# nunofachada/cl_ops

Hardware: AMD Instinct MI355X
Metric: Mkeys/s sorting 2^28 uint32 (satradix, 4-bit digits); achieved % of HBM roofline (higher is better)
Workload: dtype u32

## Files before the change

cl_ops_amd/csrc/hip/clo_hip_internal.h:

```cpp
#ifndef CLO_HIP_INTERNAL_H
#define CLO_HIP_INTERNAL_H

#include <stddef.h>
#include <stdint.h>

#include "clo_hip.h"

#define CLO_WS_STATUS_OFFSET 0
#define CLO_WS_EPOCH_WORD    2
#define CLO_WS_DONE_WORD     3
#define CLO_WS_TICKET_WORD   16
#define CLO_WS_MAX_PASSES    64
#define CLO_WS_HEADER_BYTES  512

struct clo_hip_env_t { unsigned max_spins; int radix_sweep; int r1_pools; int no_digits; int bitonic_merge2; };
const clo_hip_env_t* clo_hip_env();
int clo_radixw_preload();

inline bool clo_misaligned(const void* p, size_t align) { return ((uintptr_t) p & (align - 1)) != 0; }
inline bool clo_ws_misaligned(const void* ws) { return clo_misaligned(ws, CLO_HIP_WORKSPACE_ALIGN); }

#ifdef __HIPCC__
#include <hip/hip_runtime.h>

void clo_timing_begin(const char* label, hipStream_t s);
void clo_timing_end(hipStream_t s);
struct clo_timing_scope {
	hipStream_t s;
	clo_timing_scope(const char* label, hipStream_t stream) : s(stream) { clo_timing_begin(label, s); }
	~clo_timing_scope() { clo_timing_end(s); }
};

struct clo_keyx {
	unsigned long long sign, field;
	int kind;
};
template <typename E>
__device__ __forceinline__ E clo_keyx_fwd(E x, const clo_keyx& k) {
	if (k.kind == 1) return (E) (x ^ (E) k.sign);
	if (k.kind == 2) return (E) (x ^ ((x & (E) k.sign) ? (E) k.field : (E) k.sign));
	return x;
}
template <typename E>
__device__ __forceinline__ E clo_keyx_inv(E x, const clo_keyx& k) {
	if (k.kind == 1) return (E) (x ^ (E) k.sign);
	if (k.kind == 2) return (E) (x ^ ((x & (E) k.sign) ? (E) k.sign : (E) k.field));
	return x;
}
inline clo_keyx clo_keyx_make(int kind, int key_shift, int key_bits) {
	clo_keyx k = { 0, 0, 0 };
	if (kind == 1 || kind == 2) {
		k.kind = kind;
		k.sign = 1ull << (key_shift + key_bits - 1);
		k.field = (key_bits >= 64 ? ~0ull : ((1ull << key_bits) - 1ull)) << key_shift;
	}
	return k;
}

struct clo_kv_io {
	const void* keys_in;
	const unsigned* values_in;
	void* keys_out;
	unsigned* values_out;
};

size_t clo_radix4_workspace_bytes(size_t n, int elem_size, int digit_bits, int key_bits);
int clo_radix4_sort_kv(const clo_kv_io& io, void* pairs_a, void* pairs_b, size_t n, int key_size, int key_shift,
	int key_bits, int digit_bits, clo_keyx kx, void* ws, hipStream_t s);
size_t clo_radix4_partition_workspace_bytes(size_t n, int elem_size, int bits);
int clo_radix4_partition(const void* src, void* dst, size_t n, int elem_size, unsigned shift, int bits,
	unsigned long long* counts, void* ws, hipStream_t s);
int clo_radix4_sort(const void* src, void* dst, void* tmp, size_t n, int elem_size, int key_shift,
	int key_bits, int digit_bits, clo_keyx kx, const unsigned char* first_dig, void* ws, hipStream_t s);
int clo_radix4_takes_first_digits(size_t n, int elem_size, int digit_bits);
size_t clo_radix4_lds_bytes(int elem_size, int digit_bits);
int clo_radix1_applies(size_t n, int elem_size, int digit_bits);
size_t clo_radix1_workspace_bytes(size_t n, int elem_size, int key_bits);
int clo_radix1_sort(const void* src, void* dst, void* tmp, size_t n, int elem_size, int key_shift, int key_bits,
	clo_keyx kx, void* ws, unsigned* status, hipStream_t s);
int clo_bitonic_tiled_e1(void* data, size_t numel, int key_shift, int key_bits, int key_size, int key_kind, int descending, int* launches, hipStream_t s);
int clo_bitonic_tiled_e2(void* data, size_t numel, int key_shift, int key_bits, int key_size, int key_kind, int descending, int* launches, hipStream_t s);
int clo_bitonic_tiled_e4(void* data, size_t numel, int key_shift, int key_bits, int key_size, int key_kind, int descending, int* launches, hipStream_t s);
int clo_bitonic_tiled_e8(void* data, size_t numel, int key_shift, int key_bits, int key_size, int key_kind, int descending, int* launches, hipStream_t s);
size_t clo_radixw_lds_bytes(int digit_bits);
struct clo_radix_counters { unsigned* thist; unsigned* toff; unsigned* partial; unsigned* tinfo; unsigned tiles; bool big; };
int clo_radixw_launch_tilehist(const void* in, size_t n, int elem_size, int bits, unsigned shift, unsigned mask,
	const clo_radix_counters& c, clo_keyx kx, hipStream_t s);
int clo_radixw_launch_tilehist_kv(const void* keys, size_t n, int key_size, int bits, unsigned shift, unsigned mask,
	const clo_radix_counters& c, clo_keyx kx, hipStream_t s);
int clo_radixw_launch_tilehist_bytes(const unsigned char* dig, size_t n, int elem_size, int bits, unsigned mask,
	const clo_radix_counters& c, hipStream_t s);
int clo_radixw_launch_offsets(int bits, const clo_radix_counters& c, const unsigned** dbase, hipStream_t s);
size_t clo_radixw_partial_rows(size_t tiles);

#define CLO_SEG_MAX 256
struct clo_seg_tile { unsigned in_base, count_seg, out_base, seg_n; };
struct clo_seg_chunk { unsigned t0, tend, c_first, seg_last; };
struct clo_seg_pieces {
// ... 95 lines not shown
```

cl_ops_amd/csrc/hip/clo_hip_radix4.hip:

```cpp
#include <hip/hip_runtime.h>

#include <cstdlib>
#include <type_traits>

#include "clo_hip.h"
#include "clo_hip_internal.h"
#include "clo_hip_radix_rank.h"

namespace {

template <int KB> struct kv_key;
template <> struct kv_key<1> { typedef uint8_t type; };
template <> struct kv_key<2> { typedef uint16_t type; };
template <> struct kv_key<4> { typedef uint32_t type; };

template <int KB, int ITEMS>
__device__ __forceinline__ void kv_load_pairs(const clo_kv_io& kv, size_t at, unsigned valid, bool aligned, uint64_t (&pair)[ITEMS]) {
	typedef typename kv_key<KB>::type K;
	const K* kp = reinterpret_cast<const K*>(kv.keys_in) + at;
	K k[ITEMS];
	unsigned v[ITEMS];
	if (valid == (unsigned) ITEMS) {
		load_blocked<K, ITEMS>(kp, k, aligned);
		if (kv.values_in) {
			load_blocked<unsigned, ITEMS>(kv.values_in + at, v, aligned);
		} else {
			#pragma unroll
			for (int i = 0; i < ITEMS; ++i) v[i] = (unsigned) at + (unsigned) i;
		}
	} else {
		#pragma unroll
		for (int i = 0; i < ITEMS; ++i) {
			k[i] = (unsigned) i < valid ? kp[i] : (K) 0;
			v[i] = (unsigned) i < valid ? (kv.values_in ? kv.values_in[at + i] : (unsigned) at + (unsigned) i) : 0u;
		}
	}
	#pragma unroll
	for (int i = 0; i < ITEMS; ++i) pair[i] = ((uint64_t) k[i] << 32) | v[i];
}

template <int KB>
__device__ __forceinline__ void kv_store_pair(const clo_kv_io& kv, unsigned gi, uint64_t e) {
	typedef typename kv_key<KB>::type K;
	if (kv.keys_out) reinterpret_cast<K*>(kv.keys_out)[gi] = (K) (e >> 32);
	kv.values_out[gi] = (unsigned) e;
}

template <typename E, int LB, int HB, bool BIG, bool DIG = false, bool SEG = false, int KV_IN = 0, int KV_OUT = 0>
__global__ __launch_bounds__((pair_shape<E, BIG>::THREADS), (pair_shape<E, BIG>::THREADS >= 1024 ? 8 : 6))
void clo_radix4_pair_kernel(const E* __restrict__ in, E* __restrict__ out, size_t n,
	unsigned shift, unsigned mask_lo, unsigned mask_hi,
	const unsigned* __restrict__ thist, const unsigned* __restrict__ toff, const unsigned* __restrict__ dbase,
	const unsigned* __restrict__ tinfo, int aligned,
	clo_keyx kx_in, clo_keyx kx_out, unsigned char* __restrict__ dig_out = nullptr, unsigned next_shift = 0,
	const clo_seg_tile* __restrict__ tdesc = nullptr, const E* __restrict__ in2 = nullptr, clo_kv_io kv = clo_kv_io()) {
	static_assert((KV_IN == 0 && KV_OUT == 0) || (sizeof(E) == 8 && !SEG), "key-value passes: 8-byte pairs, one array");

	constexpr int THREADS = pair_shape<E, BIG>::THREADS;
	constexpr int ITEMS = pair_shape<E, BIG>::ITEMS;
	constexpr int TILE = THREADS * ITEMS;
	constexpr int WAVES = THREADS / 64;
	constexpr int R2 = 1 << (LB + HB);
	constexpr int HMAX = pc_words<(LB > HB ? LB : HB)>::H;
	static_assert(R2 <= 256 && R2 <= THREADS, "one thread per combined digit, scanned by the first four waves");

	__shared__ __attribute__((aligned(16))) E s_stage[TILE];
	constexpr bool ALIAS = pair_shape<E, BIG>::ALIAS;
	__shared__ unsigned s_end[ALIAS ? 1 : THREADS * PC_END_STRIDE];
	__shared__ unsigned s_wtot[WAVES][HMAX];
	__shared__ __attribute__((aligned(16))) unsigned s_wbase[WAVES][HMAX];
	__shared__ unsigned s_delta[R2];
	__shared__ unsigned s_w4[4];

	const unsigned tid = threadIdx.x, lane = tid & 63u, wave = tid >> 6;
	const unsigned per_xcd = SEG ? (unsigned) ((n + 7) / 8) : (unsigned) ((n + (size_t) TILE * 8 - 1) / ((size_t) TILE * 8));
	const unsigned tile = (blockIdx.x & 7u) * per_xcd + (blockIdx.x >> 3);
	size_t base = (size_t) tile * TILE;
	unsigned count, n32;
	if constexpr (SEG) {
		if (tile >= (unsigned) n) return;
		const clo_seg_tile td = tdesc[tile];
		base = (size_t) td.in_base;
		count = td.count_seg & 0xffffu;
		n32 = td.seg_n;
		out += td.out_base;
		if constexpr (DIG) dig_out += td.out_base;
		dbase += (size_t) ((td.count_seg >> 16) & 0x7fffu) * R2;
		if (td.count_seg >> 31) in = in2;
	} else {
		if (base >= n) return;
		count = (n - base) < (size_t) TILE ? (unsigned) (n - base) : (unsigned) TILE;
		n32 = n > 0xffffffffull ? 0xffffffffu : (unsigned) n;
	}
	const bool full = count == (unsigned) TILE;
	const unsigned tbase = tid * ITEMS;
	const unsigned mask2 = (mask_hi << LB) | mask_lo;

	__builtin_amdgcn_s_setprio(3);
	unsigned h2 = 0, goff = 0;
	if (tid < (unsigned) R2) {
		h2 = thist[(size_t) tile * R2 + tid];
		goff = toff[(size_t) tile * R2 + tid];
		if (dbase) goff += dbase[tid];
	}
	E key[ITEMS];
	if constexpr (KV_IN != 0) {
		kv_load_pairs<KV_IN, ITEMS>(kv, base + tbase, full ? (unsigned) ITEMS : (count > tbase ? count - tbase : 0u), aligned != 0, key);
	} else if (full) {
		if constexpr (SEG) load_blocked_unaligned<E, ITEMS>(in + base + tbase, key);
		else load_blocked<E, ITEMS>(in + base + tbase, key, aligned != 0);
	} else {
		#pragma unroll
		for (int i = 0; i < ITEMS; ++i) key[i] = (tbase + i < count) ? in[base + tbase + i] : (E) 0;
	}
	__builtin_amdgcn_s_setprio(0);
	if (kx_in.kind) {
		#pragma unroll
		for (int i = 0; i < ITEMS; ++i) key[i] = clo_keyx_fwd<E>(key[i], kx_in);
	}
	{
		const unsigned incl2 = clo_wave_scan_inclusive<unsigned>(h2, lane);
		if (lane == 63 && wave < 4) s_w4[wave] = incl2;
		if (tid < (unsigned) R2) s_delta[tid] = goff - (incl2 - h2);
	}

	const bool single = tinfo[tile] != 0u;

	if (!single) {
		pc_local_split<E, LB, THREADS, ITEMS, HMAX, pc_no_mid, pc_no_counted, ALIAS>(key, shift, mask_lo, count, s_stage, s_end, s_wtot, s_wbase);
	} else {
		if (full) {
			constexpr int PER = ITEMS * (int) sizeof(E) >= 16 ? 16 / (int) sizeof(E) : ITEMS;
			typedef E vec16 __attribute__((ext_vector_type(PER)));
			#pragma unroll
			for (int k = 0; k < ITEMS / PER; ++k) {
				vec16 t;
				#pragma unroll
				for (int q = 0; q < PER; ++q) t[q] = key[k * PER + q];
				*reinterpret_cast<vec16*>(&s_stage[tbase + k * PER]) = t;
			}
		} else {
			#pragma unroll
			for (int i = 0; i < ITEMS; ++i) if (tbase + i < count) s_stage[tbase + i] = key[i];
		}
		clo_lds_barrier();
	}

	if (tid < (unsigned) R2) {
		unsigned before = 0;
		#pragma unroll
		for (unsigned w = 0; w < 4; ++w) if (w < wave) before += s_w4[w];
		s_delta[tid] -= before;
	}
	if (single) {
		__syncthreads();
	} else if (mask_hi != 0) {
		if (full) {
			constexpr int PER = ITEMS * (int) sizeof(E) >= 16 ? 16 / (int) sizeof(E) : ITEMS;
			typedef E vec16 __attribute__((ext_vector_type(PER)));
			#pragma unroll
			for (int k = 0; k < ITEMS / PER; ++k) {
				const vec16 t = *reinterpret_cast<const vec16*>(&s_stage[tbase + k * PER]);
				#pragma unroll
				for (int q = 0; q < PER; ++q) key[k * PER + q] = t[q];
			}
		} else {
			#pragma unroll
			for (int i = 0; i < ITEMS; ++i) if (tbase + i < count) key[i] = s_stage[tbase + i];
		}
		pc_local_split<E, HB, THREADS, ITEMS, HMAX, pc_no_mid, pc_no_counted, ALIAS>(key, shift + LB, mask_hi, count, s_stage, s_end, s_wtot, s_wbase);
	} else {
		__syncthreads();
	}

	constexpr int VEC = sizeof(E) >= 8 ? 1 : 4;
	typedef E vecE __attribute__((ext_vector_type(VEC)));
	typedef E vecE_u __attribute__((ext_vector_type(VEC), aligned(sizeof(E))));
	const bool dig_bytes = DIG && VEC == 4 && (next_shift & 7u) == 0u && next_shift < 8u * (unsigned) sizeof(E);
	const unsigned dig_b = next_shift >> 3;
	const unsigned dig_sel_lo = 0x0c0c0400u + dig_b * 0x0101u, dig_sel_hi = 0x04000c0cu + dig_b * 0x01010000u;
	const unsigned nbits2 = (unsigned) __builtin_popcount(mask2);
	const auto scatter = [&](auto kx_tag) {
		constexpr bool KX = decltype(kx_tag)::value;
		#pragma unroll
		for (int j = 0; j < ITEMS / VEC; ++j) {
			const unsigned p = (j * THREADS + tid) * VEC;
			if (full) {
				const vecE v = *reinterpret_cast<const vecE*>(&s_stage[p]);
				const unsigned d0 = pc_digit<E>(v[0], shift, mask2, nbits2), dl = pc_digit<E>(v[VEC - 1], shift, mask2, nbits2);
				const unsigned gi0 = p + s_delta[d0];
				if (d0 == dl && gi0 <= n32 - VEC) {
					vecE vo = v;
					if constexpr (KX) {
						#pragma unroll
						for (int k = 0; k < VEC; ++k) vo[k] = clo_keyx_inv<E>(v[k], kx_out);
					}
					if constexpr (KV_OUT != 0) kv_store_pair<KV_OUT>(kv, gi0, vo[0]);
					else *reinterpret_cast<vecE_u*>(&out[gi0]) = vo;
					if constexpr (DIG) {
						if constexpr (VEC == 4) {
							typedef unsigned u32_u __attribute__((aligned(1)));
							unsigned dg;
							if (dig_bytes)
								dg = __builtin_amdgcn_perm((unsigned) v[1], (unsigned) v[0], dig_sel_lo) | __builtin_amdgcn_perm((unsigned) v[3], (unsigned) v[2], dig_sel_hi);
							else
								dg = ((unsigned) (v[0] >> next_shift) & 255u) | (((unsigned) (v[1] >> next_shift) & 255u) << 8)
									| (((unsigned) (v[2] >> next_shift) & 255u) << 16) | ((unsigned) (v[3] >> next_shift) << 24);
							*reinterpret_cast<u32_u*>(dig_out + gi0) = dg;
						} else {
							dig_out[gi0] = (unsigned char) (v[0] >> next_shift);
						}
					}
				} else {
					#pragma unroll
					for (int k = 0; k < VEC; ++k) {
						const unsigned gi = p + k + s_delta[pc_digit<E>(v[k], shift, mask2, nbits2)];
						if (gi < n32) {
							if constexpr (KV_OUT != 0) kv_store_pair<KV_OUT>(kv, gi, KX ? clo_keyx_inv<E>(v[k], kx_out) : v[k]);
							else out[gi] = KX ? clo_keyx_inv<E>(v[k], kx_out) : v[k];
							if constexpr (DIG) dig_out[gi] = (unsigned char) (v[k] >> next_shift);
						}
					}
				}
			} else {
				#pragma unroll
				for (int k = 0; k < VEC; ++k) {
					if (p + k < count) {
						const E e = s_stage[p + k];
						const unsigned gi = p + k + s_delta[pc_digit<E>(e, shift, mask2, nbits2)];
						if (gi < n32) {
							if constexpr (KV_OUT != 0) kv_store_pair<KV_OUT>(kv, gi, KX ? clo_keyx_inv<E>(e, kx_out) : e);
							else out[gi] = KX ? clo_keyx_inv<E>(e, kx_out) : e;
							if constexpr (DIG) dig_out[gi] = (unsigned char) (e >> next_shift);
						}
					}
				}
			}
		}
	};
	if (kx_out.kind) scatter(std::true_type()); else scatter(std::false_type());
}

constexpr int SMALL_TILE = 512 * 8;
template <typename E> struct small_big { static constexpr int THREADS = 1024, ITEMS = sizeof(E) == 8 ? 8 : 16, TILE = THREADS * ITEMS; };

template <typename E, int BITS, int THREADS, int ITEMS>
__global__ __launch_bounds__(THREADS)
void clo_radix4_small_kernel(const E* in, E* out, unsigned n, unsigned key_shift, unsigned key_bits, clo_keyx kx) {
	constexpr int H = pc_words<BITS>::H;
	constexpr int WAVES = THREADS / 64;
	__shared__ __attribute__((aligned(16))) E s_stage[THREADS * ITEMS];
	__shared__ unsigned s_end[THREADS * PC_END_STRIDE];
	__shared__ unsigned s_wtot[WAVES][H];
	__shared__ __attribute__((aligned(16))) unsigned s_wbase[WAVES][H];

	const unsigned tbase = threadIdx.x * ITEMS;
	E key[ITEMS];
	#pragma unroll
	for (int i = 0; i < ITEMS; ++i) key[i] = (tbase + i < n) ? clo_keyx_fwd<E>(in[tbase + i], kx) : (E) 0;
	for (unsigned done = 0; done < key_bits; done += BITS) {
		const unsigned bits = key_bits - done < (unsigned) BITS ? key_bits - done : (unsigned) BITS;
		pc_local_split<E, BITS, THREADS, ITEMS, H>(key, key_shift + done, (1u << bits) - 1u, n,
			s_stage, s_end, s_wtot, s_wbase);
		if constexpr (ITEMS * sizeof(E) >= 16) {
			constexpr int PER = 16 / (int) sizeof(E);
			typedef E vec16 __attribute__((ext_vector_type(PER)));
			#pragma unroll
			for (int k = 0; k < ITEMS / PER; ++k) {
				const vec16 t = *reinterpret_cast<const vec16*>(&s_stage[tbase + k * PER]);
				#pragma unroll
				for (int q = 0; q < PER; ++q) key[k * PER + q] = t[q];
			}
		} else {
			#pragma unroll
			for (int i = 0; i < ITEMS; ++i) if (tbase + i < n) key[i] = s_stage[tbase + i];
		}
	}
	#pragma unroll
	for (int i = 0; i < ITEMS; ++i) if (tbase + i < n) out[tbase + i] = clo_keyx_inv<E>(key[i], kx);
}


struct rp_layout { size_t thist, toff, partial, tinfo, dig, total, tiles; bool big; };

rp_layout rp_make_layout(size_t n, int elem_size, int pass_bits, bool digits = true) {
	rp_layout L;
	const size_t R2 = (size_t) 1 << pass_bits;
	L.big = clo_radix_big_tiles(n, elem_size);
	const size_t tile = clo_pair_tile_elems(elem_size, L.big);
	L.tiles = (n + tile - 1) / tile;
	if (L.tiles == 0) L.tiles = 1;
	const size_t per = L.tiles * R2 * sizeof(unsigned);
	L.thist = CLO_WS_HEADER_BYTES;
	L.toff = L.thist + per;
	L.partial = L.toff + per;
	L.tinfo = L.partial + ((clo_radixw_partial_rows(L.tiles) * R2 * sizeof(unsigned) + 255) & ~(size_t) 255);
	L.total = L.tinfo + ((L.tiles * sizeof(unsigned) + 255) & ~(size_t) 255);
	L.dig = 0;
	if (digits && clo_radix_digit_stream(n, elem_size)) {
		L.dig = L.total;
		L.total += (n + 255) & ~(size_t) 255;
	}
	return L;
}

template <typename Layout>
clo_radix_counters rp_counters(void* ws, const Layout& L, size_t tiles) {
	char* w = (char*) ws;
	return { (unsigned*) (w + L.thist), (unsigned*) (w + L.toff), (unsigned*) (w + L.partial), (unsigned*) (w + L.tinfo), (unsigned) tiles, L.big };
}

struct rp_digits { unsigned shift, mask_lo, mask_hi, mask, next_shift; };

template <int LB, int HB>
rp_digits rp_pass_digits(int p, int key_shift, int key_bits) {
	constexpr int PB = LB + HB;
	const int rem = key_bits - p * PB;
	const int bits = rem < PB ? rem : PB;
	const int lo_bits = bits < LB ? bits : LB, hi_bits = bits - lo_bits;
	rp_digits d;
	d.shift = (unsigned) (key_shift + p * PB);
	d.mask_lo = (1u << lo_bits) - 1u;
	d.mask_hi = (1u << hi_bits) - 1u;
	d.mask = (d.mask_hi << LB) | d.mask_lo;
	d.next_shift = d.shift + PB;
	return d;
}

template <typename E, int LB, int HB, bool SEG = false, int KB = 0>
void rp_launch_pass(const clo_radix_counters& c, const rp_digits& d, const E* in, E* out, size_t n, const unsigned* dbase, int aligned,
	clo_keyx kx_in, clo_keyx kx_out, unsigned char* dig_out, hipStream_t s, const clo_seg_tile* tdesc = nullptr, const E* in2 = nullptr,
	bool kv_in = false, bool kv_out = false, const clo_kv_io& kv = clo_kv_io()) {
	const unsigned tiles = SEG ? (unsigned) n : c.tiles;
	const auto launch = [&](auto big, auto dig, auto kvi, auto kvo) {
		constexpr bool BIG = decltype(big)::value, DIG = decltype(dig)::value;
		hipLaunchKernelGGL((clo_radix4_pair_kernel<E, LB, HB, BIG, DIG, SEG, decltype(kvi)::value, decltype(kvo)::value>),
			dim3((tiles + 7u) / 8u * 8u), dim3(pair_shape<E, BIG>::THREADS), 0, s,
			in, out, n, d.shift, d.mask_lo, d.mask_hi, c.thist, c.toff, dbase, c.tinfo, aligned, kx_in, kx_out, dig_out, d.next_shift, tdesc, in2, kv);
	};
	const auto shape = [&](auto kvi, auto kvo) {
		constexpr bool BIG_OK = sizeof(E) >= 4, DIG_OK = BIG_OK && LB == 4 && HB == 4 && decltype(kvo)::value == 0;
		if constexpr (DIG_OK) {
			if (c.big && dig_out) { launch(std::true_type(), std::true_type(), kvi, kvo); return; }
		}
		if constexpr (BIG_OK) {
			if (c.big) { launch(std::true_type(), std::false_type(), kvi, kvo); return; }
		}
		launch(std::false_type(), std::false_type(), kvi, kvo);
	};
	typedef std::integral_constant<int, 0> plain;
	typedef std::integral_constant<int, KB> key;
	if (kv_in && kv_out) shape(key(), key());
	else if (kv_in) shape(key(), plain());
	else if (kv_out) shape(plain(), key());
	else shape(plain(), plain());
}

int kv_unpack(const uint64_t* pairs, const clo_kv_io& io, size_t n, int key_size, hipStream_t s);

template <typename E, int LB, int HB, int KB = 0>
int rp_sort_impl(const E* src, E* dst, E* tmp, size_t n, int key_shift, int key_bits, clo_keyx kx, const unsigned char* first_dig,
	const clo_kv_io& kv, void* ws, hipStream_t s) {
	constexpr int PB = LB + HB;
	const int passes = (key_bits + PB - 1) / PB;
	const rp_layout L = rp_make_layout(n, (int) sizeof(E), PB);
	const clo_radix_counters c = rp_counters(ws, L, L.tiles);
	const bool no_dig = clo_hip_env()->no_digits != 0;
	constexpr bool DIG_OK = LB == 4 && HB == 4 && sizeof(E) >= 4;
	unsigned char* dig = (DIG_OK && L.dig != 0 && passes > 1 && !no_dig) ? (unsigned char*) ws + L.dig : nullptr;
	const clo_keyx kx_none = { 0, 0, 0 };
	const bool split_after = KB != 0 && passes == 1 && (kv.keys_out == kv.keys_in || (const void*) kv.values_out == (const void*) kv.values_in);
	const bool kv_aligned = (uintptr_t) kv.keys_in % 16 == 0 && (uintptr_t) kv.values_in % 16 == 0;

	hipError_t e;

	const bool inplace_odd = (dst == src) && (passes % 2 == 1);
	const E* cur_in = src;
	for (int p = 0; p < passes; ++p) {
		E* cur_out;
		if (inplace_odd) cur_out = (p % 2 == 0) ? tmp : dst;
		else cur_out = ((passes - 1 - p) % 2 == 0) ? dst : tmp;
		const bool kv_in = KB != 0 && p == 0, kv_out = KB != 0 && p + 1 == passes && !split_after;
		const rp_digits d = rp_pass_digits<LB, HB>(p, key_shift, key_bits);
		{
			clo_timing_scope timing("radix_hist", s);
			const unsigned char* hist_bytes = (dig && p > 0) ? dig : ((DIG_OK && c.big && p == 0 && kx.kind == 0) ? first_dig : nullptr);
			const int st = kv_in ? clo_radixw_launch_tilehist_kv(kv.keys_in, n, KB, PB, d.shift, d.mask, c, kx, s)
				: hist_bytes ? clo_radixw_launch_tilehist_bytes(hist_bytes, n, (int) sizeof(E), PB, d.mask, c, s)
				: clo_radixw_launch_tilehist(cur_in, n, (int) sizeof(E), PB, d.shift, d.mask, c, p == 0 ? kx : kx_none, s);
			if (st != 0) return st;
		}
		const unsigned* dbase = nullptr;
		{
			clo_timing_scope timing("radix_offsets", s);
			const int st = clo_radixw_launch_offsets(PB, c, &dbase, s);
			if (st != 0) return st;
		}
		{
			clo_timing_scope timing("radix_pass", s);
			const int aligned = kv_in ? (int) kv_aligned : (int) ((uintptr_t) cur_in % 16 == 0);
			rp_launch_pass<E, LB, HB, false, KB>(c, d, cur_in, cur_out, n, dbase, aligned, p == 0 ? kx : kx_none, p + 1 == passes ? kx : kx_none,
				p + 1 < passes ? dig : nullptr, s, nullptr, nullptr, kv_in, kv_out, kv);
		}
		cur_in = cur_out;
	}
	e = hipGetLastError();
	if (e != hipSuccess) return (int) e;
	if (inplace_odd) {
		e = hipMemcpyAsync(dst, tmp, n * sizeof(E), hipMemcpyDeviceToDevice, s);
		if (e != hipSuccess) return (int) e;
	}
	if constexpr (KB != 0) {
		if (split_after) return kv_unpack(dst, kv, n, KB, s);
	}
	return 0;
}

template <typename E>
int rp_dispatch(const void* src, void* dst, void* tmp, size_t n, int key_shift, int key_bits, int digit_bits,
	clo_keyx kx, const unsigned char* first_dig, void* ws, hipStream_t s) {
	#define CLO_RP(LB, HB) return rp_sort_impl<E, LB, HB>((const E*) src, (E*) dst, (E*) tmp, n, key_shift, key_bits, kx, first_dig, clo_kv_io(), ws, s)
	switch (digit_bits) {
		case 1: CLO_RP(1, 1);
		case 2: CLO_RP(2, 2);
		case 3: CLO_RP(3, 3);
		case 4: CLO_RP(4, 4);
		case 5: CLO_RP(3, 2);
		case 6: CLO_RP(3, 3);
		case 7: CLO_RP(4, 3);
		case 8: CLO_RP(4, 4);
		default: return CLO_HIP_EUNSUPPORTED;
	}
	#undef CLO_RP
}

template <int R, int R2>
__global__ __launch_bounds__(256)
void clo_radix4_counts_kernel(const unsigned* __restrict__ thist, unsigned tiles, unsigned long long* __restrict__ counts) {
	constexpr int G = 256 / R;
	__shared__ unsigned long long s_part[G][R];
	const unsigned tid = threadIdx.x, d = tid % R, g = tid / R;
	unsigned long long c = 0;
	for (unsigned t = g; t < tiles; t += G) c += thist[(size_t) t * R2 + d];
	s_part[g][d] = c;
	__syncthreads();
	if (tid < (unsigned) R) {
		unsigned long long tot = 0;
		#pragma unroll
		for (int k = 0; k < G; ++k) tot += s_part[k][tid];
		counts[tid] = tot;
	}
}

template <int R, int R2>
__global__ __launch_bounds__(256)
void clo_radix4_counts_from_bases_kernel(const unsigned* __restrict__ dbase, unsigned n, unsigned long long* __restrict__ counts) {
	const unsigned d = threadIdx.x;
	if (d < (unsigned) R) counts[d] = (unsigned long long) ((d + 1u < (unsigned) R2 ? dbase[d + 1u] : n) - dbase[d]);
}

template <typename E, int BITS, int LB, int HB>
int r4_partition_impl(const E* src, E* dst, size_t n, unsigned shift, unsigned long long* counts, void* ws, hipStream_t s) {
	constexpr unsigned R = 1u << BITS;
	constexpr int PB = LB + HB;
	constexpr bool TWO = BITS > 3;
	static_assert(TWO ? PB == BITS : (LB == BITS && HB == BITS), "see above");
	const rp_layout L = rp_make_layout(n, (int) sizeof(E), PB, false);
	const clo_radix_counters c = rp_counters(ws, L, L.tiles);
	const clo_keyx kx_none = { 0, 0, 0 };
	hipError_t e = hipMemsetAsync(ws, 0, CLO_WS_HEADER_BYTES, s);
	if (e != hipSuccess) return (int) e;
	clo_timing_scope timing("msd_partition", s);
	const rp_digits d = rp_pass_digits<LB, HB>(0, (int) shift, BITS);
	int st = clo_radixw_launch_tilehist(src, n, (int) sizeof(E), PB, d.shift, d.mask, c, kx_none, s);
	if (st != 0) return st;
	const unsigned* dbase = nullptr;
	st = clo_radixw_launch_offsets(PB, c, &dbase, s);
	if (st != 0) return st;
	if (counts) {
		if (dbase) hipLaunchKernelGGL((clo_radix4_counts_from_bases_kernel<R, (1 << PB)>), dim3(1), dim3(256), 0, s, dbase, (unsigned) n, counts);
		else hipLaunchKernelGGL((clo_radix4_counts_kernel<R, (1 << PB)>), dim3(1), dim3(256), 0, s, c.thist, c.tiles, counts);
	}
	rp_launch_pass<E, LB, HB>(c, d, src, dst, n, dbase, (int) ((uintptr_t) src % 16 == 0), kx_none, kx_none, nullptr, s);
	return (int) hipGetLastError();
}

struct rp_seg_layout { size_t thist, toff, partial, tinfo, tdesc, cdesc, dig, total, tile, max_tiles, max_chunks; bool big; };

rp_seg_layout rp_make_seg_layout(size_t n, int nseg, int elem_size) {
	rp_seg_layout L;
	const size_t R2 = 256;
	L.big = clo_radix_big_tiles(n, elem_size);
	L.tile = clo_pair_tile_elems(elem_size, L.big);
	clo_radixw_seg_bounds(n, CLO_SEG_MAX, nseg, L.tile, &L.max_tiles, &L.max_chunks);
	const size_t per = L.max_tiles * R2 * sizeof(unsigned);
	const auto up = [](size_t x) { return (x + 255) & ~(size_t) 255; };
	L.thist = CLO_WS_HEADER_BYTES;
	L.toff = L.thist + per;
	L.partial = L.toff + per;
	L.tinfo = L.partial + up(clo_radixw_partial_rows_seg(L.max_chunks, (size_t) nseg) * R2 * sizeof(unsigned));
	L.tdesc = L.tinfo + up(L.max_tiles * sizeof(unsigned));
	L.cdesc = L.tdesc + 2 * up(L.max_tiles * sizeof(clo_seg_tile));
	L.total = L.cdesc + 2 * up(L.max_chunks * sizeof(clo_seg_chunk));
	L.dig = 0;
	if (clo_radix_digit_stream(n, elem_size)) {
		L.dig = L.total;
		L.total += up(n);
	}
	return L;
}

template <typename E>
int rp_sort_seg_impl(const E* src, const E* src2, E* a, E* b, size_t n, const size_t* seg_counts, int nseg,
	const size_t* piece_n, const size_t* piece_base, const int* piece_seg, const int* piece_src, int npieces, int key_shift, int key_bits, void* ws,
	hipStream_t s, int* result_in_b) {
	constexpr int LB = 4, HB = 4, PB = 8;
	const int passes = (key_bits + PB - 1) / PB;
	const rp_seg_layout L = rp_make_seg_layout(n, nseg, (int) sizeof(E));
	const clo_radix_counters c = rp_counters(ws, L, 0);
	const auto up = [](size_t x) { return (x + 255) & ~(size_t) 255; };
	size_t seg_base[CLO_SEG_MAX];
	int seg_id[CLO_SEG_MAX];
	{
		size_t at = 0;
		for (int k = 0; k < nseg; ++k) { seg_base[k] = at; seg_id[k] = k; at += seg_counts[k]; }
	}
	clo_seg_tables sg0, sg;
	sg.tiles = (const clo_seg_tile*) ((char*) ws + L.tdesc);
	sg.chunks = (const clo_seg_chunk*) ((char*) ws + L.cdesc);
	sg.nseg = (unsigned) nseg;
	{
		clo_timing_scope timing("radix_seg_tables", s);
		int st = clo_radixw_seg_build(seg_counts, seg_base, seg_id, nullptr, nseg, nseg, L.tile, (clo_seg_tile*) sg.tiles, (clo_seg_chunk*) sg.chunks, &sg.ntiles, &sg.nchunks, s);
		if (st != 0) return st;
		sg0 = sg;
		if (npieces > 0) {
			sg0.tiles = (const clo_seg_tile*) ((char*) ws + L.tdesc + up(L.max_tiles * sizeof(clo_seg_tile)));
			sg0.chunks = (const clo_seg_chunk*) ((char*) ws + L.cdesc + up(L.max_chunks * sizeof(clo_seg_chunk)));
			st = clo_radixw_seg_build(piece_n, piece_base, piece_seg, piece_src, npieces, nseg, L.tile, (clo_seg_tile*) sg0.tiles, (clo_seg_chunk*) sg0.chunks, &sg0.ntiles, &sg0.nchunks, s);
			if (st != 0) return st;
		}
	}
	*result_in_b = passes % 2;
	if (sg.ntiles == 0) return 0;
	if (sg.ntiles > L.max_tiles || sg.nchunks > L.max_chunks || sg0.ntiles > L.max_tiles || sg0.nchunks > L.max_chunks)
		return CLO_HIP_EWORKSPACE;
	unsigned char* dig = (L.dig != 0 && passes > 1) ? (unsigned char*) ws + L.dig : nullptr;
	const clo_keyx kx_none = { 0, 0, 0 };
	const E* cur_in = src;
	for (int p = 0; p < passes; ++p) {
		const clo_seg_tables& sgp = p == 0 ? sg0 : sg;
		E* cur_out = p % 2 == 0 ? b : a;
		const rp_digits d = rp_pass_digits<LB, HB>(p, key_shift, key_bits);
		{
			clo_timing_scope timing("radix_hist", s);
			const int st = (dig && p > 0)
				? clo_radixw_launch_tilehist_bytes_seg(dig, sgp, (int) sizeof(E), PB, d.mask, c, s)
				: clo_radixw_launch_tilehist_seg(cur_in, p == 0 ? src2 : nullptr, sgp, (int) sizeof(E), PB, d.shift, d.mask, c, s);
			if (st != 0) return st;
		}
		const unsigned* dbase = nullptr;
		{
			clo_timing_scope timing("radix_offsets", s);
			const int st = clo_radixw_launch_offsets_seg(PB, c, sgp, &dbase, s);
			if (st != 0) return st;
		}
		{
			clo_timing_scope timing("radix_pass", s);
			rp_launch_pass<E, LB, HB, true>(c, d, cur_in, cur_out, (size_t) sgp.ntiles, dbase, 0, kx_none, kx_none, p + 1 < passes ? dig : nullptr, s,
				sgp.tiles, p == 0 ? src2 : nullptr);
		}
		cur_in = cur_out;
	}
	return (int) hipGetLastError();
}

template <typename E>
int small_dispatch(const void* src, void* dst, size_t n, int key_shift, int key_bits, int digit_bits, clo_keyx kx, hipStream_t s) {
	clo_timing_scope timing("radix_small", s);
	#define CLO_SMALL(B) case B: \
		if (n <= (size_t) SMALL_TILE) \
			hipLaunchKernelGGL((clo_radix4_small_kernel<E, B, 512, 8>), dim3(1), dim3(512), 0, s, \
				(const E*) src, (E*) dst, (unsigned) n, (unsigned) key_shift, (unsigned) key_bits, kx); \
		else if (n <= (size_t) 1024 * 8) \
			hipLaunchKernelGGL((clo_radix4_small_kernel<E, B, 1024, 8>), dim3(1), dim3(1024), 0, s, \
				(const E*) src, (E*) dst, (unsigned) n, (unsigned) key_shift, (unsigned) key_bits, kx); \
		else \
			hipLaunchKernelGGL((clo_radix4_small_kernel<E, B, small_big<E>::THREADS, small_big<E>::ITEMS>), dim3(1), dim3(small_big<E>::THREADS), 0, s, \
				(const E*) src, (E*) dst, (unsigned) n, (unsigned) key_shift, (unsigned) key_bits, kx); \
		break
	switch (digit_bits) {
		CLO_SMALL(1); CLO_SMALL(2); CLO_SMALL(3); CLO_SMALL(4);
		default: return CLO_HIP_EUNSUPPORTED;
	}
	#undef CLO_SMALL
	return (int) hipGetLastError();
}

constexpr int KV_PACK_THREADS = 256;

template <typename K>
__global__ __launch_bounds__(KV_PACK_THREADS)
void clo_radix_kv_pack_kernel(const K* __restrict__ keys, const unsigned* __restrict__ values, uint64_t* __restrict__ pairs, size_t n) {
	for (size_t i = (size_t) blockIdx.x * KV_PACK_THREADS + threadIdx.x; i < n; i += (size_t) gridDim.x * KV_PACK_THREADS)
		pairs[i] = ((uint64_t) keys[i] << 32) | (values ? values[i] : (unsigned) i);
}

template <typename K>
__global__ __launch_bounds__(KV_PACK_THREADS)
void clo_radix_kv_unpack_kernel(const uint64_t* __restrict__ pairs, K* __restrict__ keys, unsigned* __restrict__ values, size_t n) {
	for (size_t i = (size_t) blockIdx.x * KV_PACK_THREADS + threadIdx.x; i < n; i += (size_t) gridDim.x * KV_PACK_THREADS) {
		const uint64_t e = pairs[i];
		if (keys) keys[i] = (K) (e >> 32);
		values[i] = (unsigned) e;
	}
}

unsigned kv_pack_grid(size_t n) {
	const size_t g = (n + KV_PACK_THREADS - 1) / KV_PACK_THREADS;
	return (unsigned) (g < 8192 ? (g ? g : 1) : 8192);
}

int kv_pack(const clo_kv_io& io, uint64_t* pairs, size_t n, int key_size, hipStream_t s) {
	clo_timing_scope timing("radix_kv_pack", s);
	#define CLO_KVP(K) hipLaunchKernelGGL((clo_radix_kv_pack_kernel<K>), dim3(kv_pack_grid(n)), dim3(KV_PACK_THREADS), 0, s, (const K*) io.keys_in, io.values_in, pairs, n)
	switch (key_size) {
		case 1: CLO_KVP(uint8_t); break;
		case 2: CLO_KVP(uint16_t); break;
		case 4: CLO_KVP(uint32_t); break;
		default: return CLO_HIP_EUNSUPPORTED;
	}
	#undef CLO_KVP
	return (int) hipGetLastError();
}

int kv_unpack(const uint64_t* pairs, const clo_kv_io& io, size_t n, int key_size, hipStream_t s) {
	clo_timing_scope timing("radix_kv_unpack", s);
	#define CLO_KVU(K) hipLaunchKernelGGL((clo_radix_kv_unpack_kernel<K>), dim3(kv_pack_grid(n)), dim3(KV_PACK_THREADS), 0, s, pairs, (K*) io.keys_out, io.values_out, n)
	switch (key_size) {
		case 1: CLO_KVU(uint8_t); break;
		case 2: CLO_KVU(uint16_t); break;
		case 4: CLO_KVU(uint32_t); break;
		default: return CLO_HIP_EUNSUPPORTED;
	}
	#undef CLO_KVU
	return (int) hipGetLastError();
}

}

static size_t r4_pair_workspace_bytes(size_t n, int elem_size, int digit_bits) {
	return (rp_make_layout(n, elem_size, digit_bits <= 4 ? 2 * digit_bits : digit_bits).total + 255) & ~(size_t) 255;
// ... 111 lines not shown
```

cl_ops_amd/csrc/hip/clo_hip_runtime.hip:

```cpp
#include <hip/hip_runtime.h>

#include <cstdio>
#include <cstring>
#include <mutex>
#include <string>
#include <vector>

#include "clo_hip.h"
#include "clo_hip_internal.h"

namespace {
struct timing_rec { std::string label; hipEvent_t e0, e1; };
std::mutex g_timing_mu;
std::vector<timing_rec> g_timing;
bool g_timing_on = false;
thread_local clo_hip_launch_observer g_observer = nullptr;
thread_local void* g_observer_user = nullptr;
}

void clo_timing_begin(const char* label, hipStream_t s) {
	if (g_observer) g_observer(g_observer_user, label, 0, (void*) s);
	if (!g_timing_on) return;
	std::lock_guard<std::mutex> lk(g_timing_mu);
	timing_rec r;
// ... 61 lines not shown

int clo_hip_set_device(int device) { return (int) hipSetDevice(device); }
int clo_hip_get_device(int* device) { return device ? (int) hipGetDevice(device) : CLO_HIP_EARGS; }

int clo_hip_get_device_props(int device, clo_hip_device_props* props) {
	if (!props) return CLO_HIP_EARGS;
	hipDeviceProp_t p;
	hipError_t e = hipGetDeviceProperties(&p, device);
	if (e != hipSuccess) return (int) e;
	memset(props, 0, sizeof(*props));
	snprintf(props->name, sizeof(props->name), "%s", p.name);
	snprintf(props->gcn_arch, sizeof(props->gcn_arch), "%s", p.gcnArchName);
	props->compute_units = p.multiProcessorCount;
	props->max_threads_per_block = p.maxThreadsPerBlock;
	props->wavefront_size = p.warpSize;
	props->lds_bytes_per_block = p.sharedMemPerBlock;
	props->global_mem_bytes = p.totalGlobalMem;
	return 0;
}

int clo_hip_stream_create(void** stream) {
	if (!stream) return CLO_HIP_EARGS;
	hipStream_t s;
	hipError_t e = hipStreamCreateWithFlags(&s, hipStreamNonBlocking);
	*stream = (e == hipSuccess) ? (void*) s : nullptr;
	return (int) e;
}
int clo_hip_stream_create_high_priority(void** stream) {
	if (!stream) return CLO_HIP_EARGS;
	int least = 0, greatest = 0;
	hipError_t e = hipDeviceGetStreamPriorityRange(&least, &greatest);
	if (e != hipSuccess) return (int) e;
	hipStream_t s;
	e = hipStreamCreateWithPriority(&s, hipStreamNonBlocking, greatest);
	*stream = (e == hipSuccess) ? (void*) s : nullptr;
	return (int) e;
}
int clo_hip_stream_destroy(void* stream) { return (int) hipStreamDestroy((hipStream_t) stream); }
int clo_hip_stream_synchronize(void* stream) { return (int) hipStreamSynchronize((hipStream_t) stream); }
int clo_hip_stream_query(void* stream) {
	const hipError_t e = hipStreamQuery((hipStream_t) stream);
	if (e == hipErrorNotReady) { (void) hipGetLastError(); return CLO_HIP_ENOTREADY; }
	return (int) e;
}

int clo_hip_malloc(void** dptr, size_t bytes) {
	if (!dptr) return CLO_HIP_EARGS;
	*dptr = nullptr;
	if (bytes == 0) bytes = 4;
	return (int) hipMalloc(dptr, bytes);
}
int clo_hip_free(void* dptr) { return dptr ? (int) hipFree(dptr) : 0; }

int clo_hip_memcpy_h2d_async(void* dst, const void* src, size_t bytes, void* stream) {
	return (int) hipMemcpyAsync(dst, src, bytes, hipMemcpyHostToDevice, (hipStream_t) stream);
}
int clo_hip_memcpy_d2h_async(void* dst, const void* src, size_t bytes, void* stream) {
	return (int) hipMemcpyAsync(dst, src, bytes, hipMemcpyDeviceToHost, (hipStream_t) stream);
}
int clo_hip_memcpy_d2d_async(void* dst, const void* src, size_t bytes, void* stream) {
	return (int) hipMemcpyAsync(dst, src, bytes, hipMemcpyDeviceToDevice, (hipStream_t) stream);
}
int clo_hip_memset_async(void* dst, int value, size_t bytes, void* stream) {
	return (int) hipMemsetAsync(dst, value, bytes, (hipStream_t) stream);
}

int clo_hip_host_register(void* host_ptr, size_t bytes) {
	if (!host_ptr || bytes == 0) return CLO_HIP_EARGS;
	return (int) hipHostRegister(host_ptr, bytes, hipHostRegisterDefault);
}
int clo_hip_host_unregister(void* host_ptr) { return host_ptr ? (int) hipHostUnregister(host_ptr) : 0; }

int clo_hip_event_create(void** event) {
	if (!event) return CLO_HIP_EARGS;
	hipEvent_t ev;
	hipError_t e = hipEventCreate(&ev);
	*event = (e == hipSuccess) ? (void*) ev : nullptr;
	return (int) e;
}
int clo_hip_event_destroy(void* event) { return event ? (int) hipEventDestroy((hipEvent_t) event) : 0; }
int clo_hip_event_record(void* event, void* stream) {
	return (int) hipEventRecord((hipEvent_t) event, (hipStream_t) stream);
}
static clo_hip_env_t g_env = { CLO_MAX_SPINS, 2, 0, 0, 1 };
static int g_env_read = 0;
void clo_hip_env_refresh(void) {
	clo_hip_env_t e = { CLO_MAX_SPINS, 2, 0, 0, 1 };
	if (const char* m = getenv("CLO_MAX_SPINS")) e.max_spins = (unsigned) strtoul(m, nullptr, 10);
	if (const char* m = getenv("CLO_RADIX_SWEEP")) e.radix_sweep = atoi(m) != 0 ? 1 : 0;
	if (const char* m = getenv("CLO_R1_POOLS")) e.r1_pools = atoi(m);
	e.no_digits = getenv("CLO_RADIX_NO_DIGITS") != nullptr;
	if (const char* m = getenv("CLO_BITONIC_MERGE2")) e.bitonic_merge2 = atoi(m);
	__atomic_store_n(&g_env.max_spins, e.max_spins, __ATOMIC_RELAXED);
	__atomic_store_n(&g_env.radix_sweep, e.radix_sweep, __ATOMIC_RELAXED);
	__atomic_store_n(&g_env.r1_pools, e.r1_pools, __ATOMIC_RELAXED);
	__atomic_store_n(&g_env.no_digits, e.no_digits, __ATOMIC_RELAXED);
	__atomic_store_n(&g_env.bitonic_merge2, e.bitonic_merge2, __ATOMIC_RELAXED);
	__atomic_store_n(&g_env_read, 1, __ATOMIC_RELEASE);
}
int clo_hip_event_synchronize(void* event) { return (int) hipEventSynchronize((hipEvent_t) event); }
int clo_hip_event_query(void* event) { return event ? (int) hipEventQuery((hipEvent_t) event) : CLO_HIP_EARGS; }
int clo_hip_event_elapsed_ms(void* start, void* stop, float* ms) {
	return ms ? (int) hipEventElapsedTime(ms, (hipEvent_t) start, (hipEvent_t) stop) : CLO_HIP_EARGS;
}
int clo_hip_stream_wait_event(void* stream, void* event) {
	return (int) hipStreamWaitEvent((hipStream_t) stream, (hipEvent_t) event, 0);
}

int clo_hip_graph_capture_begin(void* stream) {
	return (int) hipStreamBeginCapture((hipStream_t) stream, hipStreamCaptureModeThreadLocal);
}

int clo_hip_stream_is_capturing(void* stream) {
	hipStreamCaptureStatus st = hipStreamCaptureStatusNone;
	if (hipStreamIsCapturing((hipStream_t) stream, &st) != hipSuccess) { (void) hipGetLastError(); return 1; }
	return st != hipStreamCaptureStatusNone ? 1 : 0;
}

int clo_hip_graph_capture_end(void* stream, void** graph_exec) {
	if (!graph_exec) return CLO_HIP_EARGS;
	*graph_exec = nullptr;
	hipGraph_t graph = nullptr;
	hipError_t e = hipStreamEndCapture((hipStream_t) stream, &graph);
	if (e != hipSuccess) return (int) e;
	hipGraphExec_t exec = nullptr;
	e = hipGraphInstantiate(&exec, graph, nullptr, nullptr, 0);
	(void) hipGraphDestroy(graph);
	if (e != hipSuccess) return (int) e;
	*graph_exec = exec;
	return 0;
}

int clo_hip_graph_launch(void* graph_exec, void* stream) {
	return graph_exec ? (int) hipGraphLaunch((hipGraphExec_t) graph_exec, (hipStream_t) stream) : CLO_HIP_EARGS;
}

int clo_hip_graph_destroy(void* graph_exec) {
	return graph_exec ? (int) hipGraphExecDestroy((hipGraphExec_t) graph_exec) : 0;
}

const char* clo_hip_error_string(int status) {
	switch (status) {
		case 0: return "success";
		case CLO_HIP_EARGS: return "clo_hip: invalid arguments";
		case CLO_HIP_EUNSUPPORTED: return "clo_hip: unsupported type or option";
		case CLO_HIP_EWORKSPACE: return "clo_hip: workspace too small";
		case CLO_HIP_ETIMEOUT: return "clo_hip: in-kernel look-back spin timed out";
		case CLO_HIP_ENOTREADY: return "clo_hip: work on the stream is still running";
		default:
			if (status <= CLO_HIP_ERCCL) return "clo_hip: RCCL reported an error (status = CLO_HIP_ERCCL - ncclResult_t)";
			return status > 0 ? hipGetErrorString((hipError_t) status) : "clo_hip: unknown error";
	}
}

int clo_hip_check_status(void* workspace, void* stream) {
	if (!workspace) return CLO_HIP_EARGS;
	unsigned int word = 0;
	hipError_t e = hipMemcpyAsync(&word, (char*) workspace + CLO_WS_STATUS_OFFSET, sizeof(word),
		hipMemcpyDeviceToHost, (hipStream_t) stream);
	if (e != hipSuccess) return (int) e;
	e = hipStreamSynchronize((hipStream_t) stream);
	if (e != hipSuccess) return (int) e;
	return word ? CLO_HIP_ETIMEOUT : 0;
}

}

const clo_hip_env_t* clo_hip_env() {
	if (!g_env_read) clo_hip_env_refresh();
	return &g_env;
}
```

Baseline: 112,900.

## Trim radix scatter address and key-transform arithmetic with 32-bit offsets

The scatter now forms global addresses from a 32-bit byte offset when the output fits in 4 GiB, selected at launch by a new wide flag (with an env override). Key transforms are simplified into a precomputed sign/neg/pos xor form, and digit-delta lookups go through an explicit LDS pointer held in a VGPR. In the slow path, mixed-digit vectors reuse the first/last deltas and only reload per-element deltas when a middle element has a third digit. The goal is fewer VALU/SALU instructions and registers in the memory-bound scatter, at the cost of doubling template instantiations and relying on asm register hints.

```diff
diff --git a/cl_ops_amd/csrc/hip/clo_hip_internal.h b/cl_ops_amd/csrc/hip/clo_hip_internal.h
--- a/cl_ops_amd/csrc/hip/clo_hip_internal.h
+++ b/cl_ops_amd/csrc/hip/clo_hip_internal.h
@@ -13,7 +13,7 @@
 #define CLO_WS_MAX_PASSES    64
 #define CLO_WS_HEADER_BYTES  512
 
-struct clo_hip_env_t { unsigned max_spins; int radix_sweep; int r1_pools; int no_digits; int bitonic_merge2; };
+struct clo_hip_env_t { unsigned max_spins; int radix_sweep; int r1_pools; int no_digits; int bitonic_merge2; int radix_wide_addr; };
 const clo_hip_env_t* clo_hip_env();
 int clo_radixw_preload();
 
diff --git a/cl_ops_amd/csrc/hip/clo_hip_radix4.hip b/cl_ops_amd/csrc/hip/clo_hip_radix4.hip
--- a/cl_ops_amd/csrc/hip/clo_hip_radix4.hip
+++ b/cl_ops_amd/csrc/hip/clo_hip_radix4.hip
@@ -39,19 +39,34 @@
 	for (int i = 0; i < ITEMS; ++i) pair[i] = ((uint64_t) k[i] << 32) | v[i];
 }
 
-template <int KB>
+template <bool WIDE, typename T>
+__device__ __forceinline__ T* rp_at(T* base, unsigned gi) {
+	if constexpr (WIDE) return base + gi;
+	else return reinterpret_cast<T*>(reinterpret_cast<char*>(base) + gi * (unsigned) sizeof(T));
+}
+
+template <int KB, bool WIDE>
 __device__ __forceinline__ void kv_store_pair(const clo_kv_io& kv, unsigned gi, uint64_t e) {
 	typedef typename kv_key<KB>::type K;
-	if (kv.keys_out) reinterpret_cast<K*>(kv.keys_out)[gi] = (K) (e >> 32);
-	kv.values_out[gi] = (unsigned) e;
-}
+	if (kv.keys_out) *rp_at<WIDE>(reinterpret_cast<K*>(kv.keys_out), gi) = (K) (e >> 32);
+	*rp_at<WIDE>(kv.values_out, gi) = (unsigned) e;
+}
+
+template <typename E> struct rp_keyx { E sign, neg, pos; };
+template <typename E>
+__device__ __forceinline__ rp_keyx<E> rp_keyx_make(const clo_keyx& k, bool inverse) {
+	const E sign = (E) k.sign, other = k.kind == 2 ? (E) k.field : sign;
+	return { sign, inverse ? sign : other, inverse ? other : sign };
+}
+template <typename E>
+__device__ __forceinline__ E rp_keyx_apply(E x, const rp_keyx<E>& k) { return (E) (x ^ ((x & k.sign) ? k.neg : k.pos)); }
 
 template <typename E, int LB, int HB, bool BIG, bool DIG = false, bool SEG = false, int KV_IN = 0, int KV_OUT = 0>
 __global__ __launch_bounds__((pair_shape<E, BIG>::THREADS), (pair_shape<E, BIG>::THREADS >= 1024 ? 8 : 6))
 void clo_radix4_pair_kernel(const E* __restrict__ in, E* __restrict__ out, size_t n,
 	unsigned shift, unsigned mask_lo, unsigned mask_hi,
 	const unsigned* __restrict__ thist, const unsigned* __restrict__ toff, const unsigned* __restrict__ dbase,
-	const unsigned* __restrict__ tinfo, int aligned,
+	const unsigned* __restrict__ tinfo, int aligned, int wide,
 	clo_keyx kx_in, clo_keyx kx_out, unsigned char* __restrict__ dig_out = nullptr, unsigned next_shift = 0,
 	const clo_seg_tile* __restrict__ tdesc = nullptr, const E* __restrict__ in2 = nullptr, clo_kv_io kv = clo_kv_io()) {
 	static_assert((KV_IN == 0 && KV_OUT == 0) || (sizeof(E) == 8 && !SEG), "key-value passes: 8-byte pairs, one array");
@@ -115,8 +130,9 @@
 	}
 	__builtin_amdgcn_s_setprio(0);
 	if (kx_in.kind) {
+		const rp_keyx<E> kf = rp_keyx_make<E>(kx_in, false);
 		#pragma unroll
-		for (int i = 0; i < ITEMS; ++i) key[i] = clo_keyx_fwd<E>(key[i], kx_in);
+		for (int i = 0; i < ITEMS; ++i) key[i] = rp_keyx_apply<E>(key[i], kf);
 	}
 	{
 		const unsigned incl2 = clo_wave_scan_inclusive<unsigned>(h2, lane);
@@ -180,23 +196,43 @@
 	const unsigned dig_b = next_shift >> 3;
 	const unsigned dig_sel_lo = 0x0c0c0400u + dig_b * 0x0101u, dig_sel_hi = 0x04000c0cu + dig_b * 0x01010000u;
 	const unsigned nbits2 = (unsigned) __builtin_popcount(mask2);
-	const auto scatter = [&](auto kx_tag) {
-		constexpr bool KX = decltype(kx_tag)::value;
+	typedef const __attribute__((address_space(3))) unsigned* lds_words;
+	unsigned nbits_v = nbits2, delta_at = (unsigned) (uintptr_t) (lds_words) s_delta;
+	if constexpr (sizeof(E) <= 4) asm volatile("" : "+v"(nbits_v));
+	asm volatile("" : "+v"(delta_at));
+	const auto digit = [&](E e) { return pc_digit<E>(e, shift, mask2, nbits_v); };
+	const auto delta = [&](unsigned d) { return *(lds_words) (uintptr_t) (delta_at + d * 4u); };
+	const auto scatter = [&](auto kx_tag, auto wide_tag) {
+		constexpr bool KX = decltype(kx_tag)::value, WIDE = decltype(wide_tag)::value;
+		rp_keyx<E> ki = rp_keyx_make<E>(kx_out, true);
+		if constexpr (KX && sizeof(E) >= 4) asm volatile("" : "+v"(ki.neg), "+v"(ki.pos));
+		const auto put = [&](unsigned gi, E e) {
+			const E eo = KX ? rp_keyx_apply<E>(e, ki) : e;
+			if constexpr (KV_OUT != 0) kv_store_pair<KV_OUT, WIDE>(kv, gi, eo);
+			else *rp_at<WIDE>(out, gi) = eo;
+			if constexpr (DIG) *rp_at<WIDE>(dig_out, gi) = (unsigned char) (e >> next_shift);
+		};
 		#pragma unroll
 		for (int j = 0; j < ITEMS / VEC; ++j) {
 			const unsigned p = (j * THREADS + tid) * VEC;
 			if (full) {
 				const vecE v = *reinterpret_cast<const vecE*>(&s_stage[p]);
-				const unsigned d0 = pc_digit<E>(v[0], shift, mask2, nbits2), dl = pc_digit<E>(v[VEC - 1], shift, mask2, nbits2);
-				const unsigned gi0 = p + s_delta[d0];
+				const unsigned d0 = digit(v[0]), dl = digit(v[VEC - 1]);
+				const unsigned delta0 = delta(d0);
+				unsigned deltal = delta0;
+				if constexpr (VEC > 1) {
+					deltal = delta(dl);
+					asm volatile("" : "+v"(deltal));
+				}
+				const unsigned gi0 = p + delta0;
 				if (d0 == dl && gi0 <= n32 - VEC) {
 					vecE vo = v;
 					if constexpr (KX) {
 						#pragma unroll
-						for (int k = 0; k < VEC; ++k) vo[k] = clo_keyx_inv<E>(v[k], kx_out);
+						for (int k = 0; k < VEC; ++k) vo[k] = rp_keyx_apply<E>(v[k], ki);
 					}
-					if constexpr (KV_OUT != 0) kv_store_pair<KV_OUT>(kv, gi0, vo[0]);
-					else *reinterpret_cast<vecE_u*>(&out[gi0]) = vo;
+					if constexpr (KV_OUT != 0) kv_store_pair<KV_OUT, WIDE>(kv, gi0, vo[0]);
+					else *reinterpret_cast<vecE_u*>(rp_at<WIDE>(out, gi0)) = vo;
 					if constexpr (DIG) {
 						if constexpr (VEC == 4) {
 							typedef unsigned u32_u __attribute__((aligned(1)));
@@ -206,20 +242,30 @@
 							else
 								dg = ((unsigned) (v[0] >> next_shift) & 255u) | (((unsigned) (v[1] >> next_shift) & 255u) << 8)
 									| (((unsigned) (v[2] >> next_shift) & 255u) << 16) | ((unsigned) (v[3] >> next_shift) << 24);
-							*reinterpret_cast<u32_u*>(dig_out + gi0) = dg;
+							*reinterpret_cast<u32_u*>(rp_at<WIDE>(dig_out, gi0)) = dg;
 						} else {
-							dig_out[gi0] = (unsigned char) (v[0] >> next_shift);
+							*rp_at<WIDE>(dig_out, gi0) = (unsigned char) (v[0] >> next_shift);
 						}
 					}
 				} else {
+					unsigned dk[VEC], dt[VEC];
+					dt[0] = delta0;
+					dt[VEC - 1] = deltal;
+					bool own = false;
+					#pragma unroll
+					for (int k = 1; k < VEC - 1; ++k) {
+						dk[k] = digit(v[k]);
+						dt[k] = dk[k] == d0 ? delta0 : deltal;
+						own |= dk[k] != d0 && dk[k] != dl;
+					}
+					if (own) {
+						#pragma unroll
+						for (int k = 1; k < VEC - 1; ++k) dt[k] = delta(dk[k]);
+					}
 					#pragma unroll
 					for (int k = 0; k < VEC; ++k) {
-						const unsigned gi = p + k + s_delta[pc_digit<E>(v[k], shift, mask2, nbits2)];
-						if (gi < n32) {
-							if constexpr (KV_OUT != 0) kv_store_pair<KV_OUT>(kv, gi, KX ? clo_keyx_inv<E>(v[k], kx_out) : v[k]);
-							else out[gi] = KX ? clo_keyx_inv<E>(v[k], kx_out) : v[k];
-							if constexpr (DIG) dig_out[gi] = (unsigned char) (v[k] >> next_shift);
-						}
+						const unsigned gi = p + k + dt[k];
+						if (gi < n32) put(gi, v[k]);
 					}
 				}
 			} else {
@@ -227,18 +273,18 @@
 				for (int k = 0; k < VEC; ++k) {
 					if (p + k < count) {
 						const E e = s_stage[p + k];
-						const unsigned gi = p + k + s_delta[pc_digit<E>(e, shift, mask2, nbits2)];
-						if (gi < n32) {
-							if constexpr (KV_OUT != 0) kv_store_pair<KV_OUT>(kv, gi, KX ? clo_keyx_inv<E>(e, kx_out) : e);
-							else out[gi] = KX ? clo_keyx_inv<E>(e, kx_out) : e;
-							if constexpr (DIG) dig_out[gi] = (unsigned char) (e >> next_shift);
-						}
+						const unsigned gi = p + k + delta(digit(e));
+						if (gi < n32) put(gi, e);
 					}
 				}
 			}
 		}
 	};
-	if (kx_out.kind) scatter(std::true_type()); else scatter(std::false_type());
+	if (wide) {
+		if (kx_out.kind) scatter(std::true_type(), std::true_type()); else scatter(std::false_type(), std::true_type());
+	} else {
+		if (kx_out.kind) scatter(std::true_type(), std::false_type()); else scatter(std::false_type(), std::false_type());
+	}
 }
 
 constexpr int SMALL_TILE = 512 * 8;
@@ -327,16 +373,21 @@
 	return d;
 }
 
+bool rp_wide_addr(size_t out_elems, size_t elem_size) {
+	return out_elems * elem_size > ((size_t) 1 << 32) || clo_hip_env()->radix_wide_addr != 0;
+}
+
 template <typename E, int LB, int HB, bool SEG = false, int KB = 0>
-void rp_launch_pass(const clo_radix_counters& c, const rp_digits& d, const E* in, E* out, size_t n, const unsigned* dbase, int aligned,
+void rp_launch_pass(const clo_radix_counters& c, const rp_digits& d, const E* in, E* out, size_t n, size_t out_elems, const unsigned* dbase, int aligned,
 	clo_keyx kx_in, clo_keyx kx_out, unsigned char* dig_out, hipStream_t s, const clo_seg_tile* tdesc = nullptr, const E* in2 = nullptr,
 	bool kv_in = false, bool kv_out = false, const clo_kv_io& kv = clo_kv_io()) {
 	const unsigned tiles = SEG ? (unsigned) n : c.tiles;
+	const int wide = rp_wide_addr(out_elems, sizeof(E)) ? 1 : 0;
 	const auto launch = [&](auto big, auto dig, auto kvi, auto kvo) {
 		constexpr bool BIG = decltype(big)::value, DIG = decltype(dig)::value;
 		hipLaunchKernelGGL((clo_radix4_pair_kernel<E, LB, HB, BIG, DIG, SEG, decltype(kvi)::value, decltype(kvo)::value>),
 			dim3((tiles + 7u) / 8u * 8u), dim3(pair_shape<E, BIG>::THREADS), 0, s,
-			in, out, n, d.shift, d.mask_lo, d.mask_hi, c.thist, c.toff, dbase, c.tinfo, aligned, kx_in, kx_out, dig_out, d.next_shift, tdesc, in2, kv);
+			in, out, n, d.shift, d.mask_lo, d.mask_hi, c.thist, c.toff, dbase, c.tinfo, aligned, wide, kx_in, kx_out, dig_out, d.next_shift, tdesc, in2, kv);
 	};
 	const auto shape = [&](auto kvi, auto kvo) {
 		constexpr bool BIG_OK = sizeof(E) >= 4, DIG_OK = BIG_OK && LB == 4 && HB == 4 && decltype(kvo)::value == 0;
@@ -399,7 +450,7 @@
 		{
 			clo_timing_scope timing("radix_pass", s);
 			const int aligned = kv_in ? (int) kv_aligned : (int) ((uintptr_t) cur_in % 16 == 0);
-			rp_launch_pass<E, LB, HB, false, KB>(c, d, cur_in, cur_out, n, dbase, aligned, p == 0 ? kx : kx_none, p + 1 == passes ? kx : kx_none,
+			rp_launch_pass<E, LB, HB, false, KB>(c, d, cur_in, cur_out, n, n, dbase, aligned, p == 0 ? kx : kx_none, p + 1 == passes ? kx : kx_none,
 				p + 1 < passes ? dig : nullptr, s, nullptr, nullptr, kv_in, kv_out, kv);
 		}
 		cur_in = cur_out;
@@ -481,7 +532,7 @@
 		if (dbase) hipLaunchKernelGGL((clo_radix4_counts_from_bases_kernel<R, (1 << PB)>), dim3(1), dim3(256), 0, s, dbase, (unsigned) n, counts);
 		else hipLaunchKernelGGL((clo_radix4_counts_kernel<R, (1 << PB)>), dim3(1), dim3(256), 0, s, c.thist, c.tiles, counts);
 	}
-	rp_launch_pass<E, LB, HB>(c, d, src, dst, n, dbase, (int) ((uintptr_t) src % 16 == 0), kx_none, kx_none, nullptr, s);
+	rp_launch_pass<E, LB, HB>(c, d, src, dst, n, n, dbase, (int) ((uintptr_t) src % 16 == 0), kx_none, kx_none, nullptr, s);
 	return (int) hipGetLastError();
 }
 
@@ -567,7 +618,7 @@
 		}
 		{
 			clo_timing_scope timing("radix_pass", s);
-			rp_launch_pass<E, LB, HB, true>(c, d, cur_in, cur_out, (size_t) sgp.ntiles, dbase, 0, kx_none, kx_none, p + 1 < passes ? dig : nullptr, s,
+			rp_launch_pass<E, LB, HB, true>(c, d, cur_in, cur_out, (size_t) sgp.ntiles, n, dbase, 0, kx_none, kx_none, p + 1 < passes ? dig : nullptr, s,
 				sgp.tiles, p == 0 ? src2 : nullptr);
 		}
 		cur_in = cur_out;
diff --git a/cl_ops_amd/csrc/hip/clo_hip_runtime.hip b/cl_ops_amd/csrc/hip/clo_hip_runtime.hip
--- a/cl_ops_amd/csrc/hip/clo_hip_runtime.hip
+++ b/cl_ops_amd/csrc/hip/clo_hip_runtime.hip
@@ -167,20 +167,22 @@
 int clo_hip_event_record(void* event, void* stream) {
 	return (int) hipEventRecord((hipEvent_t) event, (hipStream_t) stream);
 }
-static clo_hip_env_t g_env = { CLO_MAX_SPINS, 2, 0, 0, 1 };
+static clo_hip_env_t g_env = { CLO_MAX_SPINS, 2, 0, 0, 1, 0 };
 static int g_env_read = 0;
 void clo_hip_env_refresh(void) {
-	clo_hip_env_t e = { CLO_MAX_SPINS, 2, 0, 0, 1 };
+	clo_hip_env_t e = { CLO_MAX_SPINS, 2, 0, 0, 1, 0 };
 	if (const char* m = getenv("CLO_MAX_SPINS")) e.max_spins = (unsigned) strtoul(m, nullptr, 10);
 	if (const char* m = getenv("CLO_RADIX_SWEEP")) e.radix_sweep = atoi(m) != 0 ? 1 : 0;
 	if (const char* m = getenv("CLO_R1_POOLS")) e.r1_pools = atoi(m);
 	e.no_digits = getenv("CLO_RADIX_NO_DIGITS") != nullptr;
 	if (const char* m = getenv("CLO_BITONIC_MERGE2")) e.bitonic_merge2 = atoi(m);
+	e.radix_wide_addr = getenv("CLO_RADIX_WIDE_ADDR") != nullptr;
 	__atomic_store_n(&g_env.max_spins, e.max_spins, __ATOMIC_RELAXED);
 	__atomic_store_n(&g_env.radix_sweep, e.radix_sweep, __ATOMIC_RELAXED);
 	__atomic_store_n(&g_env.r1_pools, e.r1_pools, __ATOMIC_RELAXED);
 	__atomic_store_n(&g_env.no_digits, e.no_digits, __ATOMIC_RELAXED);
 	__atomic_store_n(&g_env.bitonic_merge2, e.bitonic_merge2, __ATOMIC_RELAXED);
+	__atomic_store_n(&g_env.radix_wide_addr, e.radix_wide_addr, __ATOMIC_RELAXED);
 	__atomic_store_n(&g_env_read, 1, __ATOMIC_RELEASE);
 }
 int clo_hip_event_synchronize(void* event) { return (int) hipEventSynchronize((hipEvent_t) event); }
```

Measured after the change: 114,100, median of 6. 1.1% higher.
